# tomvanbraeckel/amv-codec-tools

Measured on AMD Instinct MI355X. Metric: AMV frames/sec/GPU (160x120 decode, bit-exact), higher is better.
Workload: dtype int32; 1 GPU; 160x120 AMV decode, 160000-frame synthetic stream per GPU, chunks resident in HBM; parallelism=frame-range x1, frames_per_gpu=160000, stream=seeded synthetic source (BASELINE.md section 4), every frame

## Files before the change

amv-codec-tools_amd/csrc/amv_reconstruct.hip:

```cpp
#include "amv_block_load.h"

namespace amv {

namespace {

struct __attribute__((aligned(4))) Px12 { uint32_t w[3]; };

constexpr int kWave = 64;
constexpr int kSegMcus = 10;
constexpr int kRowsPerGroup = 4;

__device__ __forceinline__ int mad24(int x, int w, int c) {
    int d;
    asm("v_mad_i32_i24 %0, %1, %2, %3" : "=v"(d) : "v"(x), "s"(w), "v"(c));
    return d;
}

enum RowKind { kRowPlain, kRow0, kRow4 };

template <bool kColumn, RowKind kKind = kRowPlain>
__device__ __forceinline__ void idct8(int& v0, int& v1, int& v2, int& v3, int& v4, int& v5, int& v6, int& v7) {
    constexpr int W1 = 2841, W2 = 2676, W3 = 2408, W5 = 1609, W6 = 1108, W7 = 565;
    constexpr int kBias = kKind == kRow0 ? 128 + 8192 : 128;
    constexpr int kRound = kColumn ? 4 : 0;
    constexpr int kDown = kColumn ? 3 : 0;
    constexpr int kOut = kColumn ? 14 : 8;
    int a0 = kColumn ? v0 : v0 * 2048 + kBias, a1 = kColumn ? v4 : v4 * 2048;
    const int i2 = v6, i3 = v2, i4 = v1, i5 = v7, i6 = v5, i7 = v3;
    int t;
    int a4 = mad24(i4, W1, mad24(i5, W7, kRound)) >> kDown;
    int a5 = mad24(i4, W7, mad24(i5, -W1, kRound)) >> kDown;
    int a6 = mad24(i6, W5, mad24(i7, W3, kRound)) >> kDown;
    int a7 = mad24(i6, W3, mad24(i7, -W5, kRound)) >> kDown;
    t = a0 + a1;
    a0 -= a1;
    int a2 = mad24(i3, W6, mad24(i2, -W2, kRound)) >> kDown;
    int a3 = mad24(i3, W2, mad24(i2, W6, kRound)) >> kDown;
    a1 = a4 + a6;
    a4 -= a6;
    a6 = a5 + a7;
    a5 -= a7;
    a7 = t + a3;
    t -= a3;
    a3 = a0 + a2;
    a0 -= a2;
    a2 = (181 * (a4 + a5) + 128) >> 8;
    a4 = (181 * (a4 - a5) + 128) >> 8;
    v0 = a7 + a1;
    v1 = a3 + a2;
    v2 = a0 + a4;
    v3 = t + a6;
    v4 = t - a6;
    v5 = a0 - a4;
    v6 = a3 - a2;
    v7 = a7 - a1;
    if (kKind == kRowPlain) {
        v0 >>= kOut; v1 >>= kOut; v2 >>= kOut; v3 >>= kOut; v4 >>= kOut; v5 >>= kOut; v6 >>= kOut; v7 >>= kOut;
    } else {
        v0 &= ~255; v1 &= ~255; v2 &= ~255; v3 &= ~255; v4 &= ~255; v5 &= ~255; v6 &= ~255; v7 &= ~255;
    }
}

struct QuantWords { uint32_t w[2][16]; };
constexpr QuantWords pack_quant() {
    QuantWords q{};
    for (int i = 0; i < 64; ++i) {
        q.w[0][i >> 2] |= (uint32_t)kQuantLuma[i] << (8 * (i & 3));
        q.w[1][i >> 2] |= (uint32_t)kQuantChroma[i] << (8 * (i & 3));
    }
    return q;
}
__device__ const QuantWords kQuantWords = pack_quant();

__device__ __forceinline__ int clamp_iclp(int x) { return min(max(x, -256), 255); }

constexpr uint32_t pair16(int lo, int hi) { return ((uint32_t)lo & 0xffffu) | ((uint32_t)hi << 16); }
__device__ __forceinline__ uint32_t dot2_bias(uint32_t a, uint32_t w) {
    uint32_t d;
    asm("v_dot2_i32_i16 %0, %1, %2, %3" : "=v"(d) : "v"(a), "s"(w), "v"(32768u));
    return d;
}

__device__ __forceinline__ uint32_t sat_pair(uint32_t yy, uint32_t cc) {
    uint32_t sum, d;
    asm("v_pk_add_i16 %0, %1, %2" : "=v"(sum) : "v"(yy), "v"(cc));
    asm("v_sat_pk_u8_i16 %0, %1" : "=v"(d) : "v"(sum));
    return d;
}

}

template <bool kRound, int kRows>
__global__ __launch_bounds__(kWave * kRows) void amv_reconstruct_kernel(
    SyncSinks in, const uint32_t* __restrict__ nmcu_ok, uint32_t n, FrameSel sel,
    FrameGeom g, PieceMap pm, uint32_t flags, uint8_t* __restrict__ out) {
    constexpr uint32_t kPitchY = kSegMcus * 16, kPitchC = kSegMcus * 8;
    __shared__ __attribute__((aligned(16))) int16_t s_all[kRows][16 * kPitchY + 2 * 8 * kPitchC + 64];
    static_assert((16 * kPitchY + 2 * 8 * kPitchC) * 2 == kSegImageBytes, "the planes reuse the image");
    const uint32_t lane = threadIdx.x & 63u, wave = (uint32_t)__builtin_amdgcn_readfirstlane((int)(threadIdx.x >> 6));
    const uint32_t nseg = pm.nseg;
    uint32_t item0, row_group, seg;
    if (!locate_piece(pm, blockIdx.x, item0, row_group, seg)) return;
    const uint32_t my = row_group * kRows + wave;
    if (my >= g.mcu_rows) return;
    int16_t* const s_mem = s_all[wave];
    int16_t* const s_y = s_mem;
    int16_t* const s_u = s_mem + 16 * kPitchY;
    int16_t* const s_v = s_u + 8 * kPitchC;
    uint8_t* const s_img = reinterpret_cast<uint8_t*>(s_mem);

    uint32_t qw[16];
    {
        const uint4* q4 = reinterpret_cast<const uint4*>(kQuantWords.w[lane % 6u >= 4u ? 1 : 0]);
#pragma unroll
        for (int i = 0; i < 4; ++i) {
            const uint4 q = q4[i];
            qw[4 * i] = q.x; qw[4 * i + 1] = q.y; qw[4 * i + 2] = q.z; qw[4 * i + 3] = q.w;
        }
    }
    for (uint32_t item = item0;; item += piece_stride(pm)) {
    uint32_t f, slot;
    if (!select_frame(sel, n, item, f, slot)) return;
    const uint32_t m0 = seg * kSegMcus;
    const uint32_t cnt = min((uint32_t)kSegMcus, g.mcu_cols - m0);

    const uint32_t ok = nmcu_ok[f];
    const uint32_t mcu0 = my * g.mcu_cols + m0;

    uint32_t c[32];
    bool skip;
    if (load_segment_blocks(in, f, slot, kRound, g, my * nseg + seg, g.mcu_rows * nseg, mcu0, cnt, ok, lane, s_img, c, skip)) {
        const uint32_t m = lane / 6u, k6 = lane % 6u;
        const bool chroma = k6 >= 4u;
        int v[64];
#pragma unroll
        for (int nat = 0; nat < 64; ++nat) {
            const int scan = kScanOfNatural[nat];
            v[nat] = coef_at(c, scan) * (int)((qw[scan >> 2] >> (8 * (scan & 3))) & 255u);
        }
        if (!(flags & kFlagZigzagFixed))
            v[kAmvlibQuirkNatural] = coef_at(c, kAmvlibQuirkScan) * (int)((qw[kAmvlibQuirkScan >> 2] >> (8 * (kAmvlibQuirkScan & 3))) & 255u);
#pragma unroll
        for (int r = 0; r < 8; ++r) {
            if (r == 0) idct8<false, kRow0>(v[0], v[1], v[2], v[3], v[4], v[5], v[6], v[7]);
            else if (r == 4) idct8<false, kRow4>(v[32], v[33], v[34], v[35], v[36], v[37], v[38], v[39]);
            else idct8<false>(v[8 * r], v[8 * r + 1], v[8 * r + 2], v[8 * r + 3], v[8 * r + 4], v[8 * r + 5], v[8 * r + 6], v[8 * r + 7]);
        }
#pragma unroll
        for (int col = 0; col < 8; ++col)
            idct8<true>(v[col], v[8 + col], v[16 + col], v[24 + col], v[32 + col], v[40 + col], v[48 + col], v[56 + col]);
        int16_t* dst = chroma ? (k6 == 4u ? s_u : s_v) + m * 8u
                              : s_y + ((k6 >> 1) * 8u) * kPitchY + m * 16u + (k6 & 1u) * 8u;
        const uint32_t pitch = chroma ? kPitchC : kPitchY;
#pragma unroll
        for (int r = 0; r < 8; ++r) {
            uint32_t w[4];
#pragma unroll
            for (int q = 0; q < 4; ++q) {
                const int lo = clamp_iclp(v[8 * r + 2 * q]);
                const int hi = clamp_iclp(v[8 * r + 2 * q + 1]);
                w[q] = __builtin_amdgcn_perm((uint32_t)hi, (uint32_t)lo, 0x05040100u);
            }
            *reinterpret_cast<uint4*>(dst + r * pitch) = make_uint4(w[0], w[1], w[2], w[3]);
        }
    }
    if (skip) return;
    seg_sync();

    const uint32_t vr = min(16u, g.height - my * 16u);
    const uint32_t px = min(cnt * 16u, g.width - m0 * 16u);
    const uint32_t groups = cnt * 4u;
    const bool all_decoded = mcu0 + cnt <= ok;
    const uint32_t pairs = (vr + 1u) >> 1;
    const uint32_t step_i2 = kWave / groups, step_gi = kWave - step_i2 * groups;
    uint32_t i2 = lane / groups, gi = lane - i2 * groups;
    uint8_t* const frame = out + (uint64_t)f * g.frame_bytes;
    const uint32_t row0 = (g.height - 1u - my * 16u) * g.stride + m0 * 48u;
    for (; i2 < pairs; i2 += step_i2, gi += step_gi) {
        if (gi >= groups) { gi -= groups; ++i2; if (i2 >= pairs) break; }
        const uint32_t lc = gi * 4u;
        uint2 ya = *reinterpret_cast<const uint2*>(s_y + (2u * i2) * kPitchY + lc);
        uint2 yb = *reinterpret_cast<const uint2*>(s_y + (2u * i2 + 1u) * kPitchY + lc);
        uint32_t uu = *reinterpret_cast<const uint32_t*>(s_u + i2 * kPitchC + (lc >> 1));
        uint32_t vv = *reinterpret_cast<const uint32_t*>(s_v + i2 * kPitchC + (lc >> 1));
        if (!all_decoded && (mcu0 + (gi >> 2)) >= ok) {
            constexpr uint32_t kDark = 0xfc00fc00u;
            ya.x = ya.y = yb.x = yb.y = kDark;
            uu = vv = 0u;
        }
        uint32_t cr[2], cg[2], cb[2];
#pragma unroll
        for (int e = 0; e < 2; ++e) {
            const uint32_t uv = __builtin_amdgcn_perm(vv, uu, e ? 0x07060302u : 0x05040100u);
            const uint32_t r = dot2_bias(uv, pair16(18, 367));
            const uint32_t gg = dot2_bias(uv, pair16(-159, -220));
            const uint32_t b = dot2_bias(uv, pair16(411, -29));
            cr[e] = __builtin_amdgcn_perm(r, r, 0x02010201u);
            cg[e] = __builtin_amdgcn_perm(gg, gg, 0x02010201u);
            cb[e] = __builtin_amdgcn_perm(b, b, 0x02010201u);
        }
        if (lc >= px) continue;
        uint32_t off = row0 - 2u * i2 * g.stride + lc * 3u;
#pragma unroll
        for (int row = 0; row < 2; ++row) {
            const uint2 yy = row ? yb : ya;
            const uint32_t b01 = sat_pair(yy.x, cb[0]), g01 = sat_pair(yy.x, cg[0]), r01 = sat_pair(yy.x, cr[0]);
            const uint32_t b23 = sat_pair(yy.y, cb[1]), g23 = sat_pair(yy.y, cg[1]), r23 = sat_pair(yy.y, cr[1]);
            const uint32_t gr = g01 | (r01 << 16);
            const uint32_t bg = b23 | (g23 << 16);
            Px12 v;
            v.w[0] = __builtin_amdgcn_perm(gr, b01, 0x01060400u);
            v.w[1] = __builtin_amdgcn_perm(bg, gr, 0x06040301u);
            v.w[2] = __builtin_amdgcn_perm(bg, r23, 0x01070500u);
            if (2u * i2 + (uint32_t)row >= vr) break;
            if (lc + 4u <= px) {
                *reinterpret_cast<Px12*>(frame + off) = v;
            } else {
#pragma unroll
                for (uint32_t q = 0; q < 9u; ++q)
                    if (q < (px - lc) * 3u) frame[off + q] = (uint8_t)(v.w[q >> 2] >> (8u * (q & 3u)));
            }
            off -= g.stride;
        }
    }
    if (!kRound) return;
    seg_sync();
    }
}

template <int kRows>
static void launch_rows(const SyncSinks& sinks, const uint32_t* nmcu_ok, uint32_t n, const FrameSel& sel, uint32_t items, const FrameGeom& g,
                        uint32_t flags, uint8_t* out, hipStream_t s) {
    const uint32_t nseg = (g.mcu_cols + kSegMcus - 1) / kSegMcus;
    const uint32_t row_groups = (g.mcu_rows + kRows - 1) / kRows;
    PieceMap pm = make_piece_map(row_groups, nseg);
    if (sel.round) {
        const uint32_t grid = set_walkers(pm, items > 512u ? 512u : items);
        hipLaunchKernelGGL((amv_reconstruct_kernel<true, kRows>), dim3(grid), dim3(kWave * kRows), 0, s, sinks, nmcu_ok, n, sel, g, pm, flags, out);
        return;
    }
    const uint32_t most = most_items(pm);
    for (uint32_t base = 0; base < items; base += most) {
        pm.item_base = base;
        const uint32_t grid = set_walkers(pm, items - base < most ? items - base : most);
        hipLaunchKernelGGL((amv_reconstruct_kernel<false, kRows>), dim3(grid), dim3(kWave * kRows), 0, s, sinks, nmcu_ok, n, sel, g, pm, flags, out);
    }
}

void launch_reconstruct(const SyncSinks& sinks, const uint32_t* nmcu_ok, uint32_t n, const FrameSel& sel, uint32_t items,
                        const FrameGeom& g, uint32_t flags, uint8_t* out, hipStream_t s) {
    if (items == 0) return;
    const uint32_t slots4 = (g.mcu_rows + 3u) / 4u * 4u, slots5 = (g.mcu_rows + 4u) / 5u * 5u;
    const uint32_t waste4 = slots4 - g.mcu_rows, waste5 = slots5 - g.mcu_rows;
    if (10u * waste4 * slots5 >= 10u * waste5 * slots4 + slots4 * slots5) launch_rows<5>(sinks, nmcu_ok, n, sel, items, g, flags, out, s);
    else launch_rows<kRowsPerGroup>(sinks, nmcu_ok, n, sel, items, g, flags, out, s);
}

__global__ __launch_bounds__(kWave * 4) void amv_expand_records_kernel(SyncSinks in, const uint32_t* __restrict__ nmcu_ok, uint32_t n,
                                                                        FrameGeom g, uint32_t nseg, int16_t* __restrict__ coef) {
    __shared__ __attribute__((aligned(16))) uint8_t s_img[4][kSegImageBytes + 128];
    const uint32_t lane = threadIdx.x & 63u, wave = threadIdx.x >> 6;
    const uint32_t segs = g.mcu_rows * nseg;
    const uint64_t pairs = (uint64_t)n * segs;
    for (uint64_t p = (uint64_t)blockIdx.x * 4u + wave; p < pairs; p += (uint64_t)gridDim.x * 4u) {
        const uint32_t f = (uint32_t)(p / segs), segidx = (uint32_t)(p % segs);
        const uint32_t m0 = (segidx % nseg) * kSegMcus;
        const uint32_t cnt = min((uint32_t)kSegMcus, g.mcu_cols - m0);
        const uint32_t mcu0 = (segidx / nseg) * g.mcu_cols + m0;
        const uint32_t ok = nmcu_ok[f];
        uint32_t c[32];
        bool skip;
        if (load_segment_blocks(in, f, f, false, g, segidx, segs, mcu0, cnt, ok, lane, s_img[wave], c, skip)) {
            const uint32_t blk = mcu0 * 6u + lane;
            if (blk >= (in.ok_in_blocks ? ok : ok * 6u)) {
#pragma unroll
                for (int i = 0; i < 32; ++i) c[i] = 0u;
            }
            uint4* d = reinterpret_cast<uint4*>(coef + ((uint64_t)f * g.blocks + blk) * 64u);
#pragma unroll
            for (int i = 0; i < 8; ++i) d[i] = make_uint4(c[4 * i], c[4 * i + 1], c[4 * i + 2], c[4 * i + 3]);
        }
        seg_sync();
    }
}

void launch_expand_records(const SyncSinks& sinks, const uint32_t* nmcu_ok, uint32_t n, const FrameGeom& g, int16_t* coef,
                           hipStream_t s) {
    const uint32_t nseg = (g.mcu_cols + kSegMcus - 1) / kSegMcus;
    const uint64_t groups = ((uint64_t)n * g.mcu_rows * nseg + 3u) / 4u;
    if (groups == 0) return;
    hipLaunchKernelGGL(amv_expand_records_kernel, dim3(groups < 65536u ? (uint32_t)groups : 65536u), dim3(kWave * 4), 0, s, sinks,
                       nmcu_ok, n, g, nseg, coef);
}

}
```

Before: 30.17 million frames/s.

## Rescale IDCT output and color math to cut pack/shift ops, add full-segment fast path

Changes the column IDCT to output values pre-scaled by 7 bits so clamping becomes a packed saturating convert plus shift, and pre-shifts chroma so the dot2 results land in the high half, removing per-channel perm extraction and using SDWA writes to merge saturated pairs. Adds a straight-line fast path for full 10-MCU segments with fully decoded rows that indexes the shared image directly, avoiding the generic group/pair iteration. The rescaling must stay bit-exact; the fast path reads s_img with a reciprocal-multiply row index and assumes specific geometry.

```diff
diff --git a/amv-codec-tools_amd/csrc/amv_reconstruct.hip b/amv-codec-tools_amd/csrc/amv_reconstruct.hip
--- a/amv-codec-tools_amd/csrc/amv_reconstruct.hip
+++ b/amv-codec-tools_amd/csrc/amv_reconstruct.hip
@@ -24,7 +24,7 @@
     constexpr int kBias = kKind == kRow0 ? 128 + 8192 : 128;
     constexpr int kRound = kColumn ? 4 : 0;
     constexpr int kDown = kColumn ? 3 : 0;
-    constexpr int kOut = kColumn ? 14 : 8;
+    constexpr int kOut = kColumn ? 7 : 8;
     int a0 = kColumn ? v0 : v0 * 2048 + kBias, a1 = kColumn ? v4 : v4 * 2048;
     const int i2 = v6, i3 = v2, i4 = v1, i5 = v7, i6 = v5, i7 = v3;
     int t;
@@ -72,20 +72,54 @@
 }
 __device__ const QuantWords kQuantWords = pack_quant();
 
-__device__ __forceinline__ int clamp_iclp(int x) { return min(max(x, -256), 255); }
+typedef short short2v __attribute__((ext_vector_type(2)));
+typedef unsigned short ushort2v __attribute__((ext_vector_type(2)));
+__device__ __forceinline__ uint32_t clamp_iclp_pair(int lo7, int hi7) {
+    const short2v p = __builtin_amdgcn_cvt_pk_i16(lo7, hi7) >> (short)7;
+    return __builtin_bit_cast(uint32_t, p);
+}
 
 constexpr uint32_t pair16(int lo, int hi) { return ((uint32_t)lo & 0xffffu) | ((uint32_t)hi << 16); }
 __device__ __forceinline__ uint32_t dot2_bias(uint32_t a, uint32_t w) {
     uint32_t d;
-    asm("v_dot2_i32_i16 %0, %1, %2, %3" : "=v"(d) : "v"(a), "s"(w), "v"(32768u));
+    asm("v_dot2_i32_i16 %0, %1, %2, %3" : "=v"(d) : "v"(a), "s"(w), "v"(32768u << 8));
     return d;
 }
 
 __device__ __forceinline__ uint32_t sat_pair(uint32_t yy, uint32_t cc) {
     uint32_t sum, d;
-    asm("v_pk_add_i16 %0, %1, %2" : "=v"(sum) : "v"(yy), "v"(cc));
+    asm("v_pk_add_i16 %0, %1, %2 op_sel:[0,1] op_sel_hi:[1,1]" : "=v"(sum) : "v"(yy), "v"(cc));
     asm("v_sat_pk_u8_i16 %0, %1" : "=v"(d) : "v"(sum));
     return d;
+}
+__device__ __forceinline__ void sat_pair_hi(uint32_t& d, uint32_t yy, uint32_t cc) {
+    uint32_t sum;
+    asm("v_pk_add_i16 %0, %1, %2 op_sel:[0,1] op_sel_hi:[1,1]" : "=v"(sum) : "v"(yy), "v"(cc));
+    asm("v_sat_pk_u8_i16_sdwa %0, %1 dst_sel:WORD_1 dst_unused:UNUSED_PRESERVE src0_sel:DWORD" : "+v"(d) : "v"(sum));
+}
+
+__device__ __forceinline__ void convert_patch(uint2 ya, uint2 yb, uint32_t uu, uint32_t vv, Px12 (&out)[2]) {
+    const uint32_t u7 = __builtin_bit_cast(uint32_t, __builtin_bit_cast(ushort2v, uu) << (unsigned short)7);
+    const uint32_t v7 = __builtin_bit_cast(uint32_t, __builtin_bit_cast(ushort2v, vv) << (unsigned short)7);
+    uint32_t cr[2], cg[2], cb[2];
+#pragma unroll
+    for (int e = 0; e < 2; ++e) {
+        const uint32_t uv = __builtin_amdgcn_perm(v7, u7, e ? 0x07060302u : 0x05040100u);
+        cr[e] = dot2_bias(uv, pair16(2 * 18, 2 * 367));
+        cg[e] = dot2_bias(uv, pair16(2 * -159, 2 * -220));
+        cb[e] = dot2_bias(uv, pair16(2 * 411, 2 * -29));
+    }
+#pragma unroll
+    for (int row = 0; row < 2; ++row) {
+        const uint2 yy = row ? yb : ya;
+        const uint32_t b01 = sat_pair(yy.x, cb[0]), r23 = sat_pair(yy.y, cr[1]);
+        uint32_t gr = sat_pair(yy.x, cg[0]), bg = sat_pair(yy.y, cb[1]);
+        sat_pair_hi(gr, yy.x, cr[0]);
+        sat_pair_hi(bg, yy.y, cg[1]);
+        out[row].w[0] = __builtin_amdgcn_perm(gr, b01, 0x01060400u);
+        out[row].w[1] = __builtin_amdgcn_perm(bg, gr, 0x06040301u);
+        out[row].w[2] = __builtin_amdgcn_perm(bg, r23, 0x01070500u);
+    }
 }
 
 }
@@ -156,11 +190,7 @@
         for (int r = 0; r < 8; ++r) {
             uint32_t w[4];
 #pragma unroll
-            for (int q = 0; q < 4; ++q) {
-                const int lo = clamp_iclp(v[8 * r + 2 * q]);
-                const int hi = clamp_iclp(v[8 * r + 2 * q + 1]);
-                w[q] = __builtin_amdgcn_perm((uint32_t)hi, (uint32_t)lo, 0x05040100u);
-            }
+            for (int q = 0; q < 4; ++q) w[q] = clamp_iclp_pair(v[8 * r + 2 * q], v[8 * r + 2 * q + 1]);
             *reinterpret_cast<uint4*>(dst + r * pitch) = make_uint4(w[0], w[1], w[2], w[3]);
         }
     }
@@ -169,16 +199,38 @@
 
     const uint32_t vr = min(16u, g.height - my * 16u);
     const uint32_t px = min(cnt * 16u, g.width - m0 * 16u);
+    const bool all_decoded = mcu0 + cnt <= ok;
+    uint8_t* const frame = out + (uint64_t)f * g.frame_bytes;
+    const uint32_t row0 = (g.height - 1u - my * 16u) * g.stride + m0 * 48u;
+    if (cnt == (uint32_t)kSegMcus && px == kPitchY && (vr == 16u || vr == 8u) && all_decoded) {
+        const int up = -(int)(2u * g.stride + 40u * 12u);
+        uint8_t* const frame1 = frame - g.stride;
+#pragma unroll
+        for (uint32_t k = 0; k < 5u; ++k) {
+            if (k * kWave >= 40u * 4u && vr == 8u) break;
+            const uint32_t t = lane + k * kWave;
+            if ((k + 1u) * kWave > 40u * 4u && vr == 8u && t >= 40u * 4u) break;
+            const uint32_t i2 = (t * 1639u) >> 16;
+            const uint8_t* const sy = s_img + 8u * t + 2u * kPitchY * i2;
+            const uint2 ya = *reinterpret_cast<const uint2*>(sy);
+            const uint2 yb = *reinterpret_cast<const uint2*>(sy + 2u * kPitchY);
+            const uint32_t uu = reinterpret_cast<const uint32_t*>(s_u)[t];
+            const uint32_t vv = reinterpret_cast<const uint32_t*>(s_v)[t];
+            Px12 o[2];
+            convert_patch(ya, yb, uu, vv, o);
+            const uint32_t off = (uint32_t)mad24((int)i2, up, (int)(row0 + 12u * t));
+            *reinterpret_cast<Px12*>(frame + off) = o[0];
+            *reinterpret_cast<Px12*>(frame1 + off) = o[1];
+        }
+    } else {
     const uint32_t groups = cnt * 4u;
-    const bool all_decoded = mcu0 + cnt <= ok;
     const uint32_t pairs = (vr + 1u) >> 1;
     const uint32_t step_i2 = kWave / groups, step_gi = kWave - step_i2 * groups;
     uint32_t i2 = lane / groups, gi = lane - i2 * groups;
-    uint8_t* const frame = out + (uint64_t)f * g.frame_bytes;
-    const uint32_t row0 = (g.height - 1u - my * 16u) * g.stride + m0 * 48u;
     for (; i2 < pairs; i2 += step_i2, gi += step_gi) {
         if (gi >= groups) { gi -= groups; ++i2; if (i2 >= pairs) break; }
         const uint32_t lc = gi * 4u;
+        if (lc >= px) continue;
         uint2 ya = *reinterpret_cast<const uint2*>(s_y + (2u * i2) * kPitchY + lc);
         uint2 yb = *reinterpret_cast<const uint2*>(s_y + (2u * i2 + 1u) * kPitchY + lc);
         uint32_t uu = *reinterpret_cast<const uint32_t*>(s_u + i2 * kPitchC + (lc >> 1));
@@ -188,30 +240,12 @@
             ya.x = ya.y = yb.x = yb.y = kDark;
             uu = vv = 0u;
         }
-        uint32_t cr[2], cg[2], cb[2];
-#pragma unroll
-        for (int e = 0; e < 2; ++e) {
-            const uint32_t uv = __builtin_amdgcn_perm(vv, uu, e ? 0x07060302u : 0x05040100u);
-            const uint32_t r = dot2_bias(uv, pair16(18, 367));
-            const uint32_t gg = dot2_bias(uv, pair16(-159, -220));
-            const uint32_t b = dot2_bias(uv, pair16(411, -29));
-            cr[e] = __builtin_amdgcn_perm(r, r, 0x02010201u);
-            cg[e] = __builtin_amdgcn_perm(gg, gg, 0x02010201u);
-            cb[e] = __builtin_amdgcn_perm(b, b, 0x02010201u);
-        }
-        if (lc >= px) continue;
+        Px12 o[2];
+        convert_patch(ya, yb, uu, vv, o);
         uint32_t off = row0 - 2u * i2 * g.stride + lc * 3u;
 #pragma unroll
         for (int row = 0; row < 2; ++row) {
-            const uint2 yy = row ? yb : ya;
-            const uint32_t b01 = sat_pair(yy.x, cb[0]), g01 = sat_pair(yy.x, cg[0]), r01 = sat_pair(yy.x, cr[0]);
-            const uint32_t b23 = sat_pair(yy.y, cb[1]), g23 = sat_pair(yy.y, cg[1]), r23 = sat_pair(yy.y, cr[1]);
-            const uint32_t gr = g01 | (r01 << 16);
-            const uint32_t bg = b23 | (g23 << 16);
-            Px12 v;
-            v.w[0] = __builtin_amdgcn_perm(gr, b01, 0x01060400u);
-            v.w[1] = __builtin_amdgcn_perm(bg, gr, 0x06040301u);
-            v.w[2] = __builtin_amdgcn_perm(bg, r23, 0x01070500u);
+            const Px12 v = o[row];
             if (2u * i2 + (uint32_t)row >= vr) break;
             if (lc + 4u <= px) {
                 *reinterpret_cast<Px12*>(frame + off) = v;
@@ -222,6 +256,7 @@
             }
             off -= g.stride;
         }
+    }
     }
     if (!kRound) return;
     seg_sync();
```

After: 29.80 million frames/s. 1.2% lower.
